# MarcoPolo/drand

Hardware: AMD Instinct MI355X
Metric: verified beacons/sec (whole node), quicknet G1 scheme (higher is better)
Workload: dtype u32 (Fp products on 14x28-bit limbs, 64-bit MAD accumulators; 12x32-bit Montgomery storage); 1 GPU; bls-unchained-g1-rfc9380 batch verify of a 1048576-round chain, 1048576 rounds per GPU; scheme=bls-unchained-g1-rfc9380, rounds_total=1048576, rounds_per_gpu=1048576, global_batch=1048576, parallelism=round-shard x1

## Files before the change

### drand_amd/csrc/fp_mul30.hpp

```cpp
#pragma once
#include <stdint.h>

#ifndef DH_HD
#define DH_HD __device__ __forceinline__
#endif
#ifndef DH_COUNT_PROD
#define DH_COUNT_PROD() ((void)0)
#endif

namespace dh {
namespace m30 {
constexpr int N = 13;
constexpr uint32_t MASK = 0x3fffffffu;
constexpr uint32_t N0 = 0x3ffcfffdu;

struct el {
  int32_t l[N];
};

DH_HD int32_t P(int i) {
  const int32_t t[N] = {-21845, -402915328, 356515836, -352321620, -252304353, 55215067, 288093811,
                        316751073, -321428361, 517541167, -375082566, -91332614, 1704210};
  return t[i];
}
DH_HD int32_t K_IN(int i) {
  const int32_t t[N] = {-192885889, -32767999, -532500185, -13403472, -35343150, 503405810, 6050829,
                        -194530918, -181768796, 433626394, -273043482, -129447912, 620336};
  return t[i];
}
DH_HD int32_t K_OUT(int i) {
  const int32_t t[N] = {196605, 405012480, 12582951, -50330895, 123255532, -496935601, -445360651,
                        370465813, -328370226, -362903204, 154517618, -251748295, 1439327};
  return t[i];
}

DH_HD int32_t sext30(uint32_t v) { return (int32_t)(v << 2) >> 2; }

#define M30_BODY(COL)                                                                    \
  int32_t Mq[N];                                                                         \
  int64_t acc = 0;                                                                       \
  _Pragma("unroll") for (int k = 0; k < N; k++) {                                        \
    COL(k, acc);                                                                         \
    _Pragma("unroll") for (int i = 0; i < k; i++) acc += (int64_t)Mq[i] * P(k - i);      \
    Mq[k] = sext30((uint32_t)acc * N0);                                                  \
    acc += (int64_t)Mq[k] * P(0);                                                        \
    acc >>= 30;                                                                          \
  }                                                                                      \
  _Pragma("unroll") for (int k = N; k < 2 * N - 1; k++) {                                \
    COL(k, acc);                                                                         \
    _Pragma("unroll") for (int i = k - (N - 1); i < N; i++) acc += (int64_t)Mq[i] * P(k - i); \
    R[k - N] = sext30((uint32_t)acc);                                                    \
    acc = (acc + (1 << 29)) >> 30;                                                       \
  }                                                                                      \
  R[N - 1] = (int32_t)acc;

DH_HD void mont_mul(int32_t R[N], const int32_t X[N], const int32_t Y[N]) {
#define COLM(k, acc)                                                                                  \
  _Pragma("unroll") for (int i = ((k) > N - 1 ? (k) - (N - 1) : 0); i <= ((k) < N - 1 ? (k) : N - 1); i++) \
      acc += (int64_t)X[i] * Y[(k) - i];
  M30_BODY(COLM)
#undef COLM
}

DH_HD void mont_sqr(int32_t R[N], const int32_t X[N]) {
  int32_t X2[N];
#pragma unroll
  for (int i = 0; i < N; i++) X2[i] = X[i] + X[i];
#define COLS(k, acc)                                                                        \
  _Pragma("unroll") for (int i = ((k) > N - 1 ? (k) - (N - 1) : 0); 2 * i < (k); i++)       \
      acc += (int64_t)X[i] * X2[(k) - i];                                                   \
  if (((k) & 1) == 0) acc += (int64_t)X[(k) / 2] * X[(k) / 2];
  M30_BODY(COLS)
#undef COLS
}

DH_HD el mul(const el& a, const el& b) {
  DH_COUNT_PROD();
  el r;
  mont_mul(r.l, a.l, b.l);
  return r;
}
DH_HD el sqr(const el& a) {
  DH_COUNT_PROD();
  el r;
  mont_sqr(r.l, a.l);
  return r;
}

DH_HD void opaque(el& a) {
#if defined(__AMDGCN__)
#pragma unroll
  for (int i = 0; i < N; i++) asm volatile("" : "+v"(a.l[i]));
#else
  (void)a;
#endif
}

DH_HD void slice(int32_t L[N], const uint32_t x[12]) {
  uint32_t c = 0;
#pragma unroll
  for (int i = 0; i < N; i++) {
    const int b = 30 * i, w = b >> 5, o = b & 31;
    const uint64_t two = (uint64_t)x[w] | ((w + 1 < 12) ? ((uint64_t)x[w + 1] << 32) : 0);
    const uint32_t t = ((uint32_t)(two >> o) & MASK) + c;
    c = (i < N - 1) ? (t + (1u << 29)) >> 30 : 0;
    L[i] = (int32_t)t - (int32_t)(c << 30);
  }
}

DH_HD void unslice(uint32_t r[12], const int32_t A[N]) {
  int32_t c = 0;
#pragma unroll
  for (int i = 0; i < N; i++) c = (A[i] + c) >> 30;
  const int32_t neg = c;
  uint32_t U[N];
  c = 0;
#pragma unroll
  for (int i = 0; i < N; i++) {
    const int32_t t = A[i] + (P(i) & neg) + c;
    U[i] = (uint32_t)t & MASK;
    c = t >> 30;
  }
#pragma unroll
  for (int j = 0; j < 12; j++) {
    const int b = 32 * j, i = b / 30, o = b % 30;
    uint64_t v = (uint64_t)U[i] >> o;
    if (i + 1 < N) v |= (uint64_t)U[i + 1] << (30 - o);
    if (i + 2 < N && 60 - o < 32) v |= (uint64_t)U[i + 2] << (60 - o);
    r[j] = (uint32_t)v;
  }
}

DH_HD el from(const uint32_t x[12]) {
  el a, k;
  slice(a.l, x);
#pragma unroll
  for (int i = 0; i < N; i++) k.l[i] = K_IN(i);
  return mul(a, k);
}

DH_HD void to(uint32_t r[12], const el& a) {
  el k;
#pragma unroll
  for (int i = 0; i < N; i++) k.l[i] = K_OUT(i);
  const el v = mul(a, k);
  unslice(r, v.l);
}

template <int W, int ODD, int RUNS>
DH_HD el pow_sched(const el& x, const uint32_t* sched, int len) {
  el tab[ODD + RUNS];
  {
    const el x2 = sqr(x);
    el t = x;
    tab[0] = t;
#pragma unroll 1
    for (int k = 1; k < ODD; k++) {
      el y = x2;
      opaque(y);
      t = mul(t, y);
      tab[k] = t;
    }
#pragma unroll 1
    for (int k = 0, r = W; k < RUNS; k++, r *= 2) {
      const el h = t;
#pragma unroll 1
      for (int j = 0; j < r; j++) t = sqr(t);
      t = mul(t, h);
      tab[ODD + k] = t;
    }
  }
  el acc = tab[sched[0]];
  uint32_t next = sched[1];
#pragma unroll 1
  for (int i = 1; i < len; i++) {
    const uint32_t op = next;
    next = sched[i + 1];
    const uint32_t nsq = op >> 8, k = op & 0xff;
    const el e = tab[k == 0xff ? 0 : k];
#pragma unroll 1
    for (uint32_t j = 0; j < nsq; j++) acc = sqr(acc);
    if (k != 0xff) acc = mul(acc, e);
  }
  return acc;
}
}
}
```

Measured before the change: 46.66 million beacons/s.

## Restructure 30-bit Montgomery product into templated multi-lane body with pinned accumulators

Replaces the macro-based Montgomery multiply/square with a templated body that can interleave L independent products (adding mont_mul2/mont_sqr2) to expose instruction-level parallelism. Empty asm pins on the accumulators constrain compiler scheduling. A bias trick folds the rounding and the top-bit correction on alternate columns into XOR/shift operations. Existing single-lane callers go through the new body. The 2-lane variants are not yet called here, so the gain relies on the pinning and rounding changes, and the pins could hurt scheduling.

Measured after the change: 48.13 million beacons/s (median of 6 runs). 1.03x the previous value.

```diff
diff --git a/drand_amd/csrc/fp_mul30.hpp b/drand_amd/csrc/fp_mul30.hpp
--- a/drand_amd/csrc/fp_mul30.hpp
+++ b/drand_amd/csrc/fp_mul30.hpp
@@ -36,42 +36,97 @@
 
 DH_HD int32_t sext30(uint32_t v) { return (int32_t)(v << 2) >> 2; }
 
-#define M30_BODY(COL)                                                                    \
-  int32_t Mq[N];                                                                         \
-  int64_t acc = 0;                                                                       \
-  _Pragma("unroll") for (int k = 0; k < N; k++) {                                        \
-    COL(k, acc);                                                                         \
-    _Pragma("unroll") for (int i = 0; i < k; i++) acc += (int64_t)Mq[i] * P(k - i);      \
-    Mq[k] = sext30((uint32_t)acc * N0);                                                  \
-    acc += (int64_t)Mq[k] * P(0);                                                        \
-    acc >>= 30;                                                                          \
-  }                                                                                      \
-  _Pragma("unroll") for (int k = N; k < 2 * N - 1; k++) {                                \
-    COL(k, acc);                                                                         \
-    _Pragma("unroll") for (int i = k - (N - 1); i < N; i++) acc += (int64_t)Mq[i] * P(k - i); \
-    R[k - N] = sext30((uint32_t)acc);                                                    \
-    acc = (acc + (1 << 29)) >> 30;                                                       \
-  }                                                                                      \
-  R[N - 1] = (int32_t)acc;
+template <int L>
+DH_HD void pin(const int64_t acc[L]) {
+#if defined(__AMDGCN__)
+  if (L == 1)
+    asm volatile("" ::"v"(acc[0]));
+  else
+    asm volatile("" ::"v"(acc[0]), "v"(acc[L - 1]));
+#else
+  (void)acc;
+#endif
+}
+
+constexpr int64_t BIAS = ((int64_t)1 << 29) + ((int64_t)1 << 59);
+#define M30_MAD(A, B)                                                             \
+  {                                                                               \
+    _Pragma("unroll") for (int l = 0; l < L; l++) acc[l] += (int64_t)(A) * (B);   \
+    pin<L>(acc);                                                                  \
+  }
+template <int L, bool SQ>
+DH_HD void mont_body(int32_t* const R[L], const int32_t* const X[L], const int32_t* const Y[L]) {
+  int32_t X2[L][N], Mq[L][N];
+  int64_t acc[L];
+#pragma unroll
+  for (int l = 0; l < L; l++) {
+    acc[l] = 0;
+#pragma unroll
+    for (int i = 0; i < N; i++) X2[l][i] = SQ ? X[l][i] + X[l][i] : 0;
+  }
+#pragma unroll
+  for (int k = 0; k < 2 * N - 1; k++) {
+    const int lo = k > N - 1 ? k - (N - 1) : 0, hi = k < N - 1 ? k : N - 1;
+    if (SQ) {
+#pragma unroll
+      for (int i = lo; 2 * i < k; i++) M30_MAD(X[l][i], X2[l][k - i])
+      if ((k & 1) == 0) M30_MAD(X[l][k / 2], X[l][k / 2])
+    } else {
+#pragma unroll
+      for (int i = lo; i <= hi; i++) M30_MAD(X[l][i], Y[l][k - i])
+    }
+    if (k < N) {
+#pragma unroll
+      for (int i = 0; i < k; i++) M30_MAD(Mq[l][i], P(k - i))
+#pragma unroll
+      for (int l = 0; l < L; l++) Mq[l][k] = sext30((uint32_t)acc[l] * N0);
+      M30_MAD(Mq[l][k], P(0))
+#pragma unroll
+      for (int l = 0; l < L; l++) acc[l] >>= 30;
+    } else {
+#pragma unroll
+      for (int i = k - (N - 1); i < N; i++) M30_MAD(Mq[l][i], P(k - i))
+#pragma unroll
+      for (int l = 0; l < L; l++) {
+        if ((k - N) % 2 == 0) {
+          R[l][k - N] = sext30((uint32_t)acc[l]);
+          acc[l] = (acc[l] + BIAS) >> 30;
+        } else {
+          R[l][k - N] = sext30((uint32_t)acc[l] ^ (1u << 29));
+          acc[l] >>= 30;
+        }
+      }
+    }
+  }
+#pragma unroll
+  for (int l = 0; l < L; l++) R[l][N - 1] = (int32_t)acc[l];
+}
+#undef M30_MAD
 
 DH_HD void mont_mul(int32_t R[N], const int32_t X[N], const int32_t Y[N]) {
-#define COLM(k, acc)                                                                                  \
-  _Pragma("unroll") for (int i = ((k) > N - 1 ? (k) - (N - 1) : 0); i <= ((k) < N - 1 ? (k) : N - 1); i++) \
-      acc += (int64_t)X[i] * Y[(k) - i];
-  M30_BODY(COLM)
-#undef COLM
+  int32_t* const r[1] = {R};
+  const int32_t* const x[1] = {X};
+  const int32_t* const y[1] = {Y};
+  mont_body<1, false>(r, x, y);
 }
 
 DH_HD void mont_sqr(int32_t R[N], const int32_t X[N]) {
-  int32_t X2[N];
-#pragma unroll
-  for (int i = 0; i < N; i++) X2[i] = X[i] + X[i];
-#define COLS(k, acc)                                                                        \
-  _Pragma("unroll") for (int i = ((k) > N - 1 ? (k) - (N - 1) : 0); 2 * i < (k); i++)       \
-      acc += (int64_t)X[i] * X2[(k) - i];                                                   \
-  if (((k) & 1) == 0) acc += (int64_t)X[(k) / 2] * X[(k) / 2];
-  M30_BODY(COLS)
-#undef COLS
+  int32_t* const r[1] = {R};
+  const int32_t* const x[1] = {X};
+  mont_body<1, true>(r, x, x);
+}
+
+DH_HD void mont_mul2(int32_t R0[N], int32_t R1[N], const int32_t X0[N], const int32_t X1[N], const int32_t Y0[N],
+                     const int32_t Y1[N]) {
+  int32_t* const r[2] = {R0, R1};
+  const int32_t* const x[2] = {X0, X1};
+  const int32_t* const y[2] = {Y0, Y1};
+  mont_body<2, false>(r, x, y);
+}
+DH_HD void mont_sqr2(int32_t R0[N], int32_t R1[N], const int32_t X0[N], const int32_t X1[N]) {
+  int32_t* const r[2] = {R0, R1};
+  const int32_t* const x[2] = {X0, X1};
+  mont_body<2, true>(r, x, x);
 }
 
 DH_HD el mul(const el& a, const el& b) {
```
